# marekrams/tnac4o

Measured on AMD Instinct MI355X. Metric: PEPS-contraction ms/sweep, chimera L=2048 chi=64 (boundary-MPS sweep _setup_rhoT), lower is better.
Workload: dtype f64; 1 GPU; chimera L=2048 (Nx=Ny=16, Nc=8), synthetic couplings seed 20260004, beta=3, chi=64; one sweep = 16 rows of MPO absorb + compress_mps; one step = the sweeps of the 4 lattice rotations of one instance; parallelism=1 GPU: 4 lattice rotations of one instance interleaved on 4 HIP streams, mode=sweep

## Files before the change

include/tnpeps.h:

```cpp
#ifndef TNPEPS_H
#define TNPEPS_H
#include <stdint.h>

#ifdef __cplusplus
extern "C" {
#endif

int tn_version(void);
int tn_build_id(char* buf, int n);
int tn_stream_create_masked(const uint32_t* mask_host, int nwords, void** stream_out);
int tn_stream_destroy(void* stream);
int tn_last_error(char* buf, int n);

int tn_gemm(int64_t M, int64_t N, int64_t K, double alpha, const double* A, int64_t rsa, int64_t csa,
            const double* B, int64_t rsb, int64_t csb, double beta, double* C, int64_t rsc, int64_t csc,
            int64_t batch, int64_t bsa, int64_t bsb, int64_t bsc, void* ws, int64_t ws_bytes, void* stream);
int64_t tn_gemm_ws_bytes(int64_t M, int64_t N, int64_t K, int64_t batch);

int tn_factor_products_eligible(int64_t Z, int64_t I, int64_t J, int64_t K1, int64_t N, int64_t M, int first_batched);
int64_t tn_factor_products_ws_bytes(int64_t Z, int64_t I, int64_t J, int64_t K1, int64_t N, int first_batched);
int tn_factor_products(int64_t Z, int64_t I, int64_t J, int64_t K1, int64_t N, int64_t Mhi, int64_t Mlo, const double* P, int64_t pz,
                       int64_t pi, int64_t pk, const double* X, int64_t xk, int64_t xj, int64_t xn, const double* W, int64_t wm,
                       int64_t wq, double* Out, int64_t oz, int64_t ohi, int64_t olo, int64_t on, int first_batched, void* ws,
                       int64_t ws_bytes, void* stream);

int tn_absorb(const double* A, const double* W, double* out, int64_t Dl, int64_t pold, int64_t Dr, int64_t ba,
              int64_t po, int64_t bb, int64_t pi, int hconj, int64_t batch, int64_t bsA, int64_t bsW, int64_t bsOut,
              void* stream);

int tn_qr(double* A, int64_t rs, int64_t cs, int64_t m, int64_t n, double* Q, int64_t qrs, int64_t qcs, double* R,
          int64_t rrs, int64_t rcs, int nb, double rank_tol, int64_t* keff_host, void* ws, int64_t ws_bytes, void* stream);
int64_t tn_qr_ws_bytes(int64_t m, int64_t n, int nb);
int64_t tn_panel_orth_ws_bytes(int64_t nrows, int b);
int tn_panel_orth(const double* X, int64_t rs, int64_t cs, int64_t nrows, int b, double* Y, int64_t yrs, int64_t ycs, int method,
                  int* state9_host, double* dev_host, void* ws, int64_t ws_bytes, void* stream);
int tn_panel_stats(uint64_t* out16_host, int reset);
int tn_panel_stats_stream(uint64_t* out16_host, int reset, void* stream);
int tn_smallqr_stats(uint64_t* out4_host, int reset, void* stream);
int tn_fused_timeouts(int* count_host, void* stream);
int tn_qr_batched(double* A, int64_t rs, int64_t cs, int64_t m, int64_t n, double* Q, int64_t qrs, int64_t qcs, double* R,
                  int64_t rrs, int64_t rcs, int nb, double rank_tol, int64_t* keff_host, int64_t batch, int64_t bsA, int64_t bsQ,
                  int64_t bsR, void* ws, int64_t ws_bytes, void* stream, void* const* side_streams, int nside);

int tn_svd_trunc(const double* C, int64_t crs, int64_t ccs, int64_t k, int64_t n, int64_t Dmax, double tol, double* U,
                 int64_t urs, int64_t ucs, double* S, double* Vt, int64_t vrs, int64_t vcs, int64_t* keep_host,
                 double* discarded_host, int* sweeps_host, int* info_host, void* ws, int64_t ws_bytes, void* stream);
int tn_svdvals(const double* C, int64_t crs, int64_t ccs, int64_t k, int64_t n, double* S_host, int* sweeps_host,
               int* info_host, void* ws, int64_t ws_bytes, void* stream);
int64_t tn_svd_ws_bytes(int64_t k, int64_t n, int vectors);
int tn_svdvals_async(const double* C, int64_t crs, int64_t ccs, int64_t k, int64_t n, double* out66_dev, void* stream);
int tn_svdvals_small_batched(const int64_t* desc_dev, int64_t batch, const int64_t* desc_host, double* out66_dev, void* stream);
int tn_svd_trunc_batched(const double* C, int64_t crs, int64_t ccs, int64_t k, int64_t n, int64_t Dmax, double tol, double* U,
                         int64_t urs, int64_t ucs, double* S, double* Vt, int64_t vrs, int64_t vcs, int64_t* keep_host,
                         double* discarded_host, int* sweeps_host, int* info_host, int64_t batch, int64_t bsC, int64_t bsU,
                         int64_t bsS, int64_t bsV, void* ws, int64_t ws_bytes, void* stream);
int tn_svdvals_batched(const double* C, int64_t crs, int64_t ccs, int64_t k, int64_t n, double* S_host, int* sweeps_host,
                       int* info_host, int64_t batch, int64_t bsC, void* ws, int64_t ws_bytes, void* stream);

int tn_nfactor(const double* x, int64_t n, double* out2, void* slot8, void* stream);
int tn_normalize_pow2(double* x, int64_t n, double* out2, void* scratch, int64_t scratch_bytes, void* stream);
int tn_scale_by(double* x, int64_t n, const double* scalar_dev, void* stream);
int tn_scale_phys(double* A, int64_t Dl, int64_t p, int64_t Dr, const double* diag, int inv, void* stream);

int tn_peps_factor(const double* Es, const double* E1, const double* E4, const double* Xu, const double* Xl, const double* Xr,
                   const double* Xd, const int32_t* dmap, const int32_t* rmap, int64_t q, int64_t nl, int64_t nu, double* F,
                   void* stream);
int tn_mpo_from_factor(const double* F, const int32_t* dmap, const int32_t* rmap, int64_t q, int64_t nl, int64_t nu, int64_t pd,
                       int64_t br, double* W, void* stream);
int tn_mpo_from_factor_ops(const double* F, const int32_t* dmap, const int32_t* rmap, const double* O, int64_t nop, int64_t q, int64_t nl,
                           int64_t nu, int64_t pd, int64_t br, double* Wops, void* stream);

int tn_calc_pn(const double* T1, const double* RR, const double* F, const int32_t* dmap, const int32_t* rmap,
               const int32_t* pref, const int32_t* suf, const int32_t* lidx, const int32_t* uidx, int64_t nb,
               int64_t q, int64_t nl, int64_t nu, int64_t p, int64_t Dr, int64_t br, double* P, double* minP,
               const double* parent_log2p, double* log2p_out, void* stream);
int tn_sample_pn(const double* T1, const double* RR, const double* F, const int32_t* dmap, const int32_t* rmap, const int32_t* pref,
                 const int32_t* suf, const int32_t* lidx, const int32_t* uidx, const int32_t* perm, const int64_t* starts, int64_t ng,
// ... 161 lines not shown
```

tnac4o_amd/_lib.py:

```python
import ctypes as C
import os
import subprocess

HERE = os.path.dirname(os.path.abspath(__file__))
LIB_PATH = os.path.join(HERE, 'libtnpeps.so')
CSRC = os.path.join(HERE, 'csrc')
SOURCES = ['api.hip', 'gemm_f64.hip', 'rank_update.hip', 'factor_products.hip', 'small.hip', 'qr.hip', 'svd.hip', 'absorb.hip', 'misc.hip', 'beam.hip', 'prof.hip', 'cholqr.hip', 'smallqr.hip', 'fused.hip', 'peps.hip', 'env.hip', 'batch.hip', 'site.hip', 'chain.hip', 'beamsearch.hip', 'marginal.hip', 'sampler.hip', 'overlap.hip', 'relax.hip', 'exchange.hip', 'temper.hip', 'anneal.hip', 'rng.hip', 'droplets.hip', 'linkage.hip', 'lines.hip']

_i64, _f64, _int, _ptr = C.c_int64, C.c_double, C.c_int, C.c_void_p

SIGNATURES = {
    'tn_version': (_int, []),
    'tn_last_error': (_int, [C.c_char_p, _int]),
    'tn_build_id': (_int, [C.c_char_p, _int]),
    'tn_stream_create_masked': (_int, [C.POINTER(C.c_uint32), _int, C.POINTER(_ptr)]),
    'tn_stream_destroy': (_int, [_ptr]),
    'tn_gemm': (_int, [_i64, _i64, _i64, _f64, _ptr, _i64, _i64, _ptr, _i64, _i64, _f64, _ptr, _i64, _i64,
                       _i64, _i64, _i64, _i64, _ptr, _i64, _ptr]),
    'tn_gemm_ws_bytes': (_i64, [_i64, _i64, _i64, _i64]),
    'tn_factor_products_eligible': (_int, [_i64] * 6 + [_int]),
    'tn_factor_products_ws_bytes': (_i64, [_i64] * 5 + [_int]),
    'tn_factor_products': (_int, [_i64] * 7 + [_ptr, _i64, _i64, _i64, _ptr, _i64, _i64, _i64, _ptr, _i64, _i64, _ptr, _i64, _i64, _i64, _i64,
                                  _int, _ptr, _i64, _ptr]),
    'tn_absorb': (_int, [_ptr, _ptr, _ptr, _i64, _i64, _i64, _i64, _i64, _i64, _i64, _int, _i64, _i64, _i64, _i64, _ptr]),
    'tn_qr': (_int, [_ptr, _i64, _i64, _i64, _i64, _ptr, _i64, _i64, _ptr, _i64, _i64, _int, _f64, C.POINTER(_i64), _ptr, _i64,
              _ptr]),
    'tn_qr_ws_bytes': (_i64, [_i64, _i64, _int]),
    'tn_panel_orth_ws_bytes': (_i64, [_i64, _int]),
    'tn_panel_orth': (_int, [_ptr, _i64, _i64, _i64, _int, _ptr, _i64, _i64, _int, C.POINTER(_int), C.POINTER(_f64), _ptr, _i64, _ptr]),
    'tn_panel_stats': (_int, [C.POINTER(C.c_uint64), _int]),
    'tn_panel_stats_stream': (_int, [C.POINTER(C.c_uint64), _int, _ptr]),
    'tn_smallqr_stats': (_int, [C.POINTER(C.c_uint64), _int, _ptr]),
    'tn_fused_timeouts': (_int, [C.POINTER(_int), _ptr]),
    'tn_qr_batched': (_int, [_ptr, _i64, _i64, _i64, _i64, _ptr, _i64, _i64, _ptr, _i64, _i64, _int, _f64, C.POINTER(_i64), _i64, _i64, _i64,
                      _i64, _ptr, _i64, _ptr, C.POINTER(_ptr), _int]),
    'tn_svd_trunc': (_int, [_ptr, _i64, _i64, _i64, _i64, _i64, _f64, _ptr, _i64, _i64, _ptr, _ptr, _i64, _i64,
                            C.POINTER(_i64), C.POINTER(_f64), C.POINTER(_int), C.POINTER(_int), _ptr, _i64, _ptr]),
    'tn_svdvals': (_int, [_ptr, _i64, _i64, _i64, _i64, C.POINTER(_f64), C.POINTER(_int), C.POINTER(_int), _ptr, _i64,
                          _ptr]),
    'tn_svd_ws_bytes': (_i64, [_i64, _i64, _int]),
    'tn_svdvals_async': (_int, [_ptr, _i64, _i64, _i64, _i64, _ptr, _ptr]),
    'tn_svdvals_small_batched': (_int, [_ptr, _i64, _ptr, _ptr, _ptr]),
    'tn_svd_trunc_batched': (_int, [_ptr, _i64, _i64, _i64, _i64, _i64, _f64, _ptr, _i64, _i64, _ptr, _ptr, _i64, _i64, C.POINTER(_i64),
                             C.POINTER(_f64), C.POINTER(_int), C.POINTER(_int), _i64, _i64, _i64, _i64, _i64, _ptr, _i64, _ptr]),
    'tn_svdvals_batched': (_int, [_ptr, _i64, _i64, _i64, _i64, C.POINTER(_f64), C.POINTER(_int), C.POINTER(_int), _i64, _i64, _ptr, _i64,
                           _ptr]),
    'tn_nfactor': (_int, [_ptr, _i64, _ptr, _ptr, _ptr]),
    'tn_scale_by': (_int, [_ptr, _i64, _ptr, _ptr]),
    'tn_normalize_pow2': (_int, [_ptr, _i64, _ptr, _ptr, _i64, _ptr]),
    'tn_scale_phys': (_int, [_ptr, _i64, _i64, _i64, _ptr, _int, _ptr]),
    'tn_calc_pn': (_int, [_ptr] * 9 + [_i64] * 7 + [_ptr, _ptr, _ptr, _ptr, _ptr]),
    'tn_sample_pn': (_int, [_ptr] * 11 + [_i64, _ptr] + [_i64] * 6 + [_ptr, _ptr, _ptr, _ptr]),
    'tn_score_pn': (_int, [_ptr] * 11 + [_i64, _ptr] + [_i64] * 8 + [_ptr, _ptr, _ptr, _ptr, _ptr]),
    'tn_merge_groups': (_int, [_ptr] * 5 + [_i64, _f64, _ptr, _ptr, _ptr, _ptr]),
    'tn_mpo_from_factor_ops': (_int, [_ptr] * 4 + [_i64] * 6 + [_ptr, _ptr]),
    'tn_nfactor_batched': (_int, [_ptr, _i64, _i64, _ptr]),
    'tn_env_rr_batched': (_int, [_ptr] * 5 + [_i64] * 7 + [_ptr, _ptr]),
    'tn_env_rl_batched': (_int, [_ptr] * 3 + [_i64] * 3 + [_ptr, _ptr]),
    'tn_balance': (_int, [_ptr, _i64, _i64, _i64, _f64, _ptr, _ptr, _ptr]),
    'tn_peps_factor': (_int, [_ptr] * 9 + [_i64] * 3 + [_ptr, _ptr]),
    'tn_mpo_from_factor': (_int, [_ptr] * 3 + [_i64] * 5 + [_ptr, _ptr]),
    'tn_site_qr_ws_bytes': (_i64, [_int, _i64, _i64, _i64, _i64, _int]),
    'tn_site_qr': (_int, [_int, _ptr, _i64, _i64, _i64, _ptr, _i64, _ptr, _ptr, _f64, C.POINTER(_i64), _ptr, C.POINTER(_int), C.POINTER(_f64),
                   _int, C.POINTER(_i64), _ptr, _i64, _ptr]),
    'tn_gram_weights': (_int, [_ptr, _i64, _f64, _ptr, _ptr, _ptr]),
    'tn_rows_norm2': (_int, [_ptr, _i64, _i64, _ptr, _ptr]),
    'tn_gather_scale_rows': (_int, [_ptr, _i64, _i64, _ptr, _ptr, _ptr, _int, _ptr]),
    'tn_bond_deflate': (_int, [_int, _ptr, _i64, _i64, _ptr, _i64, _ptr, _ptr, C.POINTER(_i64), C.POINTER(_f64), _ptr, _i64, _ptr]),
    'tn_rar_ws_bytes': (_i64, [_i64] * 5),
    'tn_rar': (_int, [_ptr, _ptr, _ptr] + [_i64] * 5 + [_ptr, _ptr, _i64, _ptr]),
    'tn_env_mix_ws_bytes': (_i64, [_int] + [_i64] * 5),
    'tn_env_mix': (_int, [_int, _ptr, _ptr, _ptr] + [_i64] * 5 + [_ptr, _ptr, _i64, _ptr]),
    'tn_apply_truncation_ws_bytes': (_i64, [_i64] * 5),
    'tn_apply_truncation': (_int, [_ptr, _i64, _i64, _ptr, _i64, _i64, _i64, _ptr, _i64, _i64, _ptr, _i64, _i64, _ptr, _ptr, _ptr, _ptr, _ptr,
                            _i64, _ptr]),
    'tn_compress_mps_arena_bytes': (_i64, [_i64, C.POINTER(_i64), C.POINTER(_i64), _i64]),
# ... 82 lines not shown
    src_hash = source_hash()

    def one(s):
        src = os.path.join(CSRC, s)
        h = hh.copy()
        h.update(open(src, 'rb').read())
        extra = []
        if s == 'api.hip':
            extra = ['-DTN_SRC_HASH="%s"' % src_hash]
            h.update(src_hash.encode())
        obj = os.path.join(objdir, '%s.%s.o' % (s[:-4], h.hexdigest()[:16]))
        if not os.path.exists(obj):
            for old in os.listdir(objdir):
                if old.startswith(s[:-4] + '.') and old.endswith('.o'):
                    os.unlink(os.path.join(objdir, old))
            import tempfile
            fd, tmp = tempfile.mkstemp(prefix=s[:-4] + '.', suffix='.o.part', dir=objdir)
            os.close(fd)
            cmd = [hipcc] + flags + extra + ['-c', src, '-o', tmp]
            if verbose:
                print(' '.join(cmd), flush=True)
            try:
                subprocess.run(cmd, check=True)
                os.replace(tmp, obj)
            finally:
                if os.path.exists(tmp):
                    os.unlink(tmp)
        return obj

    with ThreadPoolExecutor(max_workers=int(os.environ.get('TN_BUILD_JOBS', '6'))) as ex:
        objs = list(ex.map(one, SOURCES))
    cmd = [hipcc, '--offload-arch=gfx950', '-shared', '-fPIC', '-Wl,--no-undefined'] + os.environ.get('TN_EXTRA_HIPCC_FLAGS', '').split() + ['-o', LIB_PATH] + objs
    if verbose:
        print(' '.join(cmd), flush=True)
    subprocess.run(cmd, check=True)
    return LIB_PATH


def _stale(L):
    buf = C.create_string_buffer(64)
    L.tn_build_id.restype, L.tn_build_id.argtypes = _int, [C.c_char_p, _int]
    L.tn_build_id(buf, 64)
    return buf.value.decode() != source_hash()


SHORT_CALLS = ('tn_gemm', 'tn_gemm_ws_bytes', 'tn_qr_ws_bytes', 'tn_svd_ws_bytes', 'tn_absorb', 'tn_nfactor', 'tn_scale_by',
               'tn_normalize_pow2', 'tn_scale_phys', 'tn_calc_pn', 'tn_sample_pn', 'tn_score_pn', 'tn_nfactor_batched', 'tn_env_rr_batched', 'tn_env_rl_batched',
               'tn_balance', 'tn_merge_groups', 'tn_svdvals_async', 'tn_rar', 'tn_rar_ws_bytes', 'tn_env_mix', 'tn_env_mix_ws_bytes',
               'tn_apply_truncation', 'tn_apply_truncation_ws_bytes', 'tn_site_qr_ws_bytes', 'tn_gram_weights', 'tn_argsort_desc', 'tn_weighted_sum', 'tn_rows_norm2', 'tn_gather_scale_rows', 'tn_peps_factor', 'tn_mpo_from_factor', 'tn_env3', 'tn_env3_ws_bytes',
               'tn_cluster_marginal', 'tn_cluster_marginal_ws_bytes', 'tn_cluster_bond_marginal', 'tn_cluster_bond_marginal_ws_bytes',
               'tn_mpo_from_factor_ops', 'tn_env3_stack', 'tn_env3_stack_ws_bytes', 'tn_stack_cell_law', 'tn_stack_cell_law_ws_bytes',
               'tn_last_error')
_lib = None
ABI_VERSION = 25


def lib():
    global _lib
    if _lib is None:
        if not os.path.exists(LIB_PATH):
            raise RuntimeError('libtnpeps.so not found at %s: run `python -c "import __graft_entry__ as g; g.build()"` '
                               '(the HIP library is the only backend; there is no CPU fallback)' % LIB_PATH)
        L = C.CDLL(LIB_PATH)
        L.tn_version.restype = _int
        if not hasattr(L, 'tn_build_id') or (_stale(L) and not os.environ.get('TN_ALLOW_STALE_LIB')):
            raise RuntimeError('libtnpeps.so was built from other sources than csrc/*.hip + include/tnpeps.h in this tree: '
                               'rebuild it with `python -c "import __graft_entry__ as g; g.build()"` -- a stale library can '
                               'disagree with the ctypes signatures declared here')
        if L.tn_version() != ABI_VERSION:
            raise RuntimeError('libtnpeps.so implements C-ABI version %d, this package binds version %d: rebuild the library'
                               % (L.tn_version(), ABI_VERSION))
        if os.environ.get('TN_PYDLL', '1') != '0':
            P = C.PyDLL(LIB_PATH)
            for name in SHORT_CALLS:
                setattr(L, name, getattr(P, name))
            L._pydll = P
        for name, (res, args) in SIGNATURES.items():
            fn = getattr(L, name)
            fn.restype, fn.argtypes = res, args
        _lib = L
    return _lib


class TnError(RuntimeError):
    pass


def check(rc):
    if rc != 0:
        buf = C.create_string_buffer(512)
        lib().tn_last_error(buf, 512)
        raise TnError('libtnpeps error %d: %s' % (rc, buf.value.decode(errors='replace')))
```

tnac4o_amd/csrc/api.hip:

```cpp
#include <stdarg.h>

#include "../../include/tnpeps.h"
#include "common.h"

namespace tn {

static thread_local char g_err[512] = "";

void set_error(const char* fmt, ...) {
    va_list ap;
    va_start(ap, fmt);
    vsnprintf(g_err, sizeof(g_err), fmt, ap);
    va_end(ap);
}
const char* get_error() { return g_err; }

}

using namespace tn;
#define ST ((hipStream_t)stream)

extern "C" {

int tn_version(void) { return 25; }

#ifndef TN_SRC_HASH
#define TN_SRC_HASH "unknown"
#endif
int tn_build_id(char* buf, int n) {
    const char* e = TN_SRC_HASH;
    const int len = (int)strlen(e);
    if (buf && n > 0) {
        const int c = len < n - 1 ? len : n - 1;
        memcpy(buf, e, c);
        buf[c] = 0;
    }
    return len;
}

void tn_profile_enable(unsigned mask) { prof_set_mask(mask); }
void tn_profile_reset(void) { prof_reset(); }
void tn_profile_sample(unsigned every) { prof_set_sample(every); }
int tn_profile_get(int family, uint64_t* calls_host, double* ms_host, double* flops_host, double* bytes_host) {
    TN_CHECK_ARG(family >= 0 && family < PROF_NFAM, "unknown kernel family");
    TN_CHECK_ARG(calls_host && ms_host && flops_host && bytes_host, "null output");
    prof_get(-1, family, calls_host, ms_host, flops_host, bytes_host);
    return 0;
}
int tn_profile_get_phase(int phase, int family, uint64_t* calls_host, double* ms_host, double* flops_host, double* bytes_host) {
    TN_CHECK_ARG(phase >= -1 && phase < PH_N, "unknown phase");
    TN_CHECK_ARG(family >= 0 && family < PROF_NFAM, "unknown kernel family");
    TN_CHECK_ARG(calls_host && ms_host && flops_host && bytes_host, "null output");
    prof_get(phase, family, calls_host, ms_host, flops_host, bytes_host);
    return 0;
}

int tn_stream_create_masked(const uint32_t* mask_host, int nwords, void** stream_out) {
    TN_CHECK_ARG(mask_host && nwords >= 1 && stream_out, "bad arguments");
    hipStream_t st = nullptr;
    const hipError_t e = hipExtStreamCreateWithCUMask(&st, (uint32_t)nwords, mask_host);
    if (e != hipSuccess) return hip_fail(e, "hipExtStreamCreateWithCUMask");
    fused_forms_disable(st);
    *stream_out = (void*)st;
    return 0;
}
int tn_stream_destroy(void* stream) {
    fused_stream_released((hipStream_t)stream);
    const hipError_t e = hipStreamDestroy((hipStream_t)stream);
    return e == hipSuccess ? 0 : hip_fail(e, "hipStreamDestroy");
}

int tn_last_error(char* buf, int n) {
    const char* e = get_error();
    int len = (int)strlen(e);
    if (buf && n > 0) {
        int c = len < n - 1 ? len : n - 1;
        memcpy(buf, e, c);
// ... 312 lines not shown
```

tnac4o_amd/csrc/chain.hip:

```cpp
#include <math.h>
#include <stdlib.h>

#include <cmath>

#include <algorithm>
#include <chrono>
#include <map>
#include <memory>
#include <mutex>
#include <vector>

#include "common.h"

namespace tn {

__global__ __launch_bounds__(256) void permute4_kernel(const double* __restrict__ in, int64_t s0, int64_t s1, int64_t s2, int64_t s3, int64_t n0,
                                                       int64_t n1, int64_t n2, int64_t n3, double* __restrict__ out) {
    const int64_t tot = n0 * n1 * n2 * n3;
    for (int64_t e = (int64_t)blockIdx.x * 256 + threadIdx.x; e < tot; e += (int64_t)gridDim.x * 256) {
        const int64_t i3 = e % n3, r = e / n3, i2 = r % n2, r2 = r / n2, i1 = r2 % n1, i0 = r2 / n1;
        out[e] = in[i0 * s0 + i1 * s1 + i2 * s2 + i3 * s3];
    }
}
static int permute4(hipStream_t st, const double* in, int64_t s0, int64_t s1, int64_t s2, int64_t s3, int64_t n0, int64_t n1, int64_t n2, int64_t n3,
// ... 591 lines not shown
            const double rank_tol = (compress && 0 < n && n < L) ? CH_RANK_TOL : 0.0;
            const M2 Cm = C;
            PassMark tm(st);
            if (compress) tm.substart();
            CH(site_right(n, &Cm, rank_tol));
            if (compress) { tm.trlap(pass_id, 0); trmark = &tm; CH(truncateC(Dmax, tol)); trmark = nullptr; }
        }
        return 0;
    }

    static bool factor_pair_fused(int64_t Z, int64_t I, int64_t J, int64_t K1, int64_t N, int64_t M, int64_t M1, int64_t N1) {
        return factor_products_on() && factor_products_fits(Z, I, J, K1, N, M) && (M1 == 0 || gemm_ws_bytes(M1, N1, K1, 1) == 0);
    }
    int gram_step_structured(M2& G, int64_t n) {
        const int64_t* fd = &facdims[7 * n];
        const int64_t Dl = fd[0], ps = fd[1], Dr = fd[2], ba = fd[3], po = fd[4], bb = fd[5], pi = fd[6];
        const double* Af = facA[n];
        const double* W = facW[n];
        const int64_t wl = po * bb * pi, wr = pi;
        const int64_t wsd = hconj ? bb * pi : 1, wtd = hconj ? 1 : bb * pi;
        const int64_t pt = hconj ? pi : po;
        const int64_t na = Dl * ba;
        Ref gpb; double* Gp = nullptr;
        CH(new_block(na * ba * Dl, gpb, Gp, "Gram (permuted)"));
        if (hconj) CH(permute4(st, G.p, ba * na, na, 1, ba, Dl, ba, ba, Dl, Gp));
        else CH(permute4(st, G.p, na, Dl * na, Dl, 1, Dl, ba, ba, Dl, Gp));
        Ref wxb; double* Wx = nullptr;
        Ref t2b; double* T2 = nullptr;
        if (factor_pair_fused(na, ba, ps, Dl, Dr, pt * bb, na * ba, ps * Dr)) {
            CH(new_block(pt * bb * ba * ps, wxb, Wx, "Wx"));
            CH(permute4(st, W, wl, wsd, wtd, wr, ba, ps, pt, bb, Wx));
            CH(new_block(na * pt * bb * Dr, t2b, T2, "Gram step T2"));
            FactorProducts f;
            f.Z = na; f.I = ba; f.J = ps; f.K1 = Dl; f.N = Dr; f.Mhi = 1; f.Mlo = pt * bb;
            f.P = Gp; f.pz = ba * Dl; f.pi = Dl; f.pk = 1;
            f.X = Af; f.xk = ps * Dr; f.xj = Dr; f.xn = 1;
            f.W = Wx; f.wm = 1; f.wq = pt * bb;
            f.Out = T2; f.oz = pt * bb * Dr; f.ohi = 0; f.olo = Dr; f.on = 1;
            CH(factor_products(st, f));
            gpb.reset();
        } else {
            Ref t1b; double* T1 = nullptr;
            CH(new_block(na * ba * ps * Dr, t1b, T1, "Gram step T1"));
            CH(mm(na * ba, ps * Dr, Dl, Gp, Dl, 1, Af, ps * Dr, 1, T1, ps * Dr, 1));
            gpb.reset();
            CH(new_block(pt * bb * ba * ps, wxb, Wx, "Wx"));
            CH(permute4(st, W, wtd, wr, wl, wsd, pt, bb, ba, ps, Wx));
            CH(new_block(na * pt * bb * Dr, t2b, T2, "Gram step T2"));
            CH(bmm(na, pt * bb, Dr, ba * ps, Wx, ba * ps, 1, 0, T1, Dr, 1, ba * ps * Dr, T2, Dr, 1, pt * bb * Dr));
        }
        Ref wyb; double* Wy = nullptr;
        CH(new_block(ps * bb * ba * pt, wyb, Wy, "Wy"));
        CH(permute4(st, W, wsd, wr, wl, wtd, ps, bb, ba, pt, Wy));
        Ref ub; double* U = nullptr;
        CH(new_block(Dl * ps * bb * bb * Dr, ub, U, "Gram step U"));
        CH(bmm(Dl, ps * bb, bb * Dr, ba * pt, Wy, ba * pt, 1, 0, T2, bb * Dr, 1, ba * pt * bb * Dr, U, bb * Dr, 1, ps * bb * bb * Dr));
        t2b.reset();
        Ref ob; double* O = nullptr;
        CH(new_block(Dr * bb * bb * Dr, ob, O, "Gram step O"));
        CH(mm(Dr, bb * bb * Dr, Dl * ps, Af, 1, Dr, U, bb * bb * Dr, 1, O, bb * bb * Dr, 1));
        ub.reset();
        M2 Gn;
        CH(new_m2(Dr * bb, Dr * bb, Gn, "Gram matrix"));
        if (hconj) CH(permute4(st, O, bb * bb * Dr, bb * Dr, 1, Dr, Dr, bb, Dr, bb, Gn.p));
        else CH(permute4(st, O, bb * Dr, bb * bb * Dr, Dr, 1, bb, Dr, bb, Dr, Gn.p));
        G = Gn;
        return 0;
    }
    int ensure_absorbed(int64_t n) {
        if (A[n].p) return 0;
        if (facA.empty() || !facA[n]) { set_error("tn_compress_mps: site %lld has neither a tensor nor its factors", (long long)n); return -1; }
        const int64_t* fd = &facdims[7 * n];
        T3 t;
        CH(new_t3(A[n].a, A[n].b, A[n].c, t, "absorbed site"));
        {
            ProfPhase ph(PH_ABSORB);
            CH(absorb(st, facA[n], facW[n], t.p, fd[0], fd[1], fd[2], fd[3], fd[4], fd[5], fd[6], hconj, 1, 0, 0, 0));
        }
        A[n] = t;
        return 0;
    }
    int attach_through_factors(int64_t n, const M2& Cm, double* Am) {
        const int64_t* fd = &facdims[7 * n];
        const int64_t Dl = fd[0], ps = fd[1], Dr = fd[2], ba = fd[3], po = fd[4], bb = fd[5], pi = fd[6], r = Cm.c;
        const int64_t pt = hconj ? pi : po;
        if (Cm.r != Dr * bb || (hconj ? po : pi) != ps) { set_error("tn_compress_mps: centre matrix does not fit the factors of site %lld", (long long)n); return -1; }
        if (factor_pair_fused(Dl, ps, bb, Dr, r, ba * pt, hconj ? Dl * ps : 0, bb * r)) {
            Ref wb; double* Wq = nullptr;
            CH(new_block(ba * pt * ps * bb, wb, Wq, "attach through the factors: W"));
            if (hconj) CH(permute4(st, facW[n], bb * pi, pi, po * bb * pi, 1, ps, bb, ba, pt, Wq));
            else CH(permute4(st, facW[n], 1, pi, po * bb * pi, bb * pi, ps, bb, ba, pt, Wq));
            FactorProducts f;
            f.Z = Dl; f.I = ps; f.J = bb; f.K1 = Dr; f.N = r; f.Mhi = ba; f.Mlo = pt;
            f.P = facA[n]; f.pz = ps * Dr; f.pi = Dr; f.pk = 1;
            f.X = Cm.p; f.xk = hconj ? bb * r : r; f.xj = hconj ? r : Dr * r; f.xn = 1;
            f.W = Wq; f.wm = 1; f.wq = ba * pt;
            f.Out = Am; f.oz = hconj ? ba * pt * r : pt * r; f.ohi = hconj ? pt * r : Dl * pt * r; f.olo = r; f.on = 1;
            return factor_products(st, f);
        }
        Ref tb; double* T = nullptr;
        CH(new_block(Dl * ps * bb * r, tb, T, "attach through the factors: T"));
        if (hconj) CH(mm(Dl * ps, bb * r, Dr, facA[n], Dr, 1, Cm.p, bb * r, 1, T, bb * r, 1));
        else CH(bmm(bb, Dl * ps, r, Dr, facA[n], Dr, 1, 0, Cm.p, r, 1, Dr * r, T, bb * r, 1, r));
        Ref wb; double* Wq = nullptr;
        CH(new_block(ba * pt * ps * bb, wb, Wq, "attach through the factors: W"));
        if (hconj) CH(permute4(st, facW[n], po * bb * pi, 1, bb * pi, pi, ba, pt, ps, bb, Wq));
// ... 504 lines not shown
    pm.lap(5);
    if ((rc = ch.variational_compress(*target, tolV, max_sweeps, lazy))) return rc;
    pm.lap(6);
    for (int64_t n = 0; n < L; ++n) {
        const T3& t = ch.A[n];
        TN_CHECK_ARG(t.numel() <= out_slot, "output slot too small for a compressed site");
        const hipError_t e = hipMemcpyAsync(out + n * out_slot, t.p, (size_t)t.numel() * 8, hipMemcpyDeviceToDevice, st);
        if (e != hipSuccess) return hip_fail(e, "copy result");
        out_dims_host[3 * n] = t.a; out_dims_host[3 * n + 1] = t.b; out_dims_host[3 * n + 2] = t.c;
    }
    pm.lap(7);
    if (overlap_host) *overlap_host = ch.overlap;
    if (discarded_host) for (int64_t i = 0; i <= L; ++i) discarded_host[i] = ch.discarded[i];
    if (schmidt_host && schmidt_len_host) {
        for (int64_t i = 0; i <= L; ++i) {
            Chain::SState& s = ch.Sst[i];
            if (s.is_lazy) {
                std::vector<double> v;
                if ((rc = ch.svdvals_host(s.lazy, v))) return rc;
                s.val = v; s.has = true; s.is_lazy = false; s.lazy = M2();
            }
            const int64_t len = s.has ? std::min<int64_t>((int64_t)s.val.size(), schmidt_pitch) : 0;
            schmidt_len_host[i] = s.has ? len : -1;
            for (int64_t j = 0; j < len; ++j) schmidt_host[i * schmidt_pitch + j] = s.val[j];
        }
    }
    if (ch.nfs_overflow) {
        set_error("tn_compress_mps: the table of normalisation factors is too small (%lld pairs): size it (2 max_sweeps + 16) L + 64", (long long)nfs_cap);
        return -3;
    }
    if (nfs_count_host) *nfs_count_host = ch.nfs_count;
    if (info_host) {
        info_host[0] = ch.reveal_error_bound;
        info_host[1] = (double)ch.reveal_fallbacks;
        info_host[2] = (double)ch.weighted_used;
        info_host[3] = (double)ar.peak();
        info_host[4] = (double)ch.bonds_before;
        info_host[5] = (double)ch.bonds_after;
        info_host[6] = 0.0;
        info_host[7] = (double)ch.gauge_skipped + 65536.0 * (double)ch.target_swapped + 131072.0 * (double)ch.var1_skipped + 262144.0 * (double)ch.attach_fused;
    }
    return 0;
}

int tn_argsort_desc(const double* w, int64_t n, int64_t* perm_out, void* stream) {
    TN_CHECK_ARG(w && perm_out, "null operand");
    return argsort_desc((hipStream_t)stream, w, n, perm_out);
}
int tn_weighted_sum(const double* a, const double* b, int64_t n, double* w_out, double* sum_out, void* stream) {
    TN_CHECK_ARG(a && b && w_out && sum_out, "null operand");
    return weighted_sum((hipStream_t)stream, a, b, n, w_out, sum_out);
}

}
```

tnac4o_amd/csrc/common.h:

```cpp
#pragma once
#include <hip/hip_runtime.h>
#include <stdint.h>
#include <stdio.h>
#include <stdlib.h>
#include <string.h>

namespace tn {

void set_error(const char* fmt, ...);
const char* get_error();

inline int hip_fail(hipError_t e, const char* what) {
    set_error("%s: %s", what, hipGetErrorString(e));
    return (int)e > 0 ? (int)e : 1;
}

#define TN_CHECK_ARG(cond, msg)                \
    do {                                       \
        if (!(cond)) {                         \
            tn::set_error("%s: %s", __func__, msg); \
            return -1;                         \
        }                                      \
    } while (0)

// ... 74 lines not shown
void prof_set_sample(unsigned n);
void prof_reset();
void prof_get(int phase, int fam, uint64_t* calls, double* ms, double* flops, double* bytes);

struct Mat {
    double* p;
    int64_t rs, cs;
};
static inline Mat mat(double* p, int64_t rs, int64_t cs) { return Mat{p, rs, cs}; }
static inline Mat sub(Mat a, int64_t i, int64_t j) { return Mat{a.p + i * a.rs + j * a.cs, a.rs, a.cs}; }
static inline Mat tr(Mat a) { return Mat{a.p, a.cs, a.rs}; }

int gemm(hipStream_t st, int64_t M, int64_t N, int64_t K, double alpha, const double* A, int64_t rsa, int64_t csa,
         const double* B, int64_t rsb, int64_t csb, double beta, double* C, int64_t rsc, int64_t csc,
         int64_t batch = 1, int64_t bsa = 0, int64_t bsb = 0, int64_t bsc = 0, double* ws = nullptr,
         int64_t ws_bytes = 0);
int64_t gemm_ws_bytes(int64_t M, int64_t N, int64_t K, int64_t batch);
struct GemmExtra {
    const int* pairs = nullptr;
    const int* skip = nullptr;
    int pw = 0, mapA = 0, mapB = 0, mapC = 0;
    int force_splitk = 0;
    bool raw_partials = false;
    int* splitk_used = nullptr;
};
int gemm_forced_split(int64_t K, int s, int64_t* kchunk);
int gemm_ex(hipStream_t st, int64_t M, int64_t N, int64_t K, double alpha, const double* A, int64_t rsa, int64_t csa,
            const double* B, int64_t rsb, int64_t csb, double beta, double* C, int64_t rsc, int64_t csc, int64_t batch,
            int64_t bsa, int64_t bsb, int64_t bsc, double* ws, int64_t ws_bytes, const GemmExtra* x);

static inline int gemm(hipStream_t st, int64_t M, int64_t N, int64_t K, double alpha, Mat A, Mat B, double beta, Mat C,
                       double* ws = nullptr, int64_t ws_bytes = 0) {
    return gemm(st, M, N, K, alpha, A.p, A.rs, A.cs, B.p, B.rs, B.cs, beta, C.p, C.rs, C.cs, 1, 0, 0, 0, ws, ws_bytes);
}
int gemm_prof_family(int64_t M, int64_t N, int64_t K, int64_t rsc, int64_t csc);

int rank_update(hipStream_t st, int64_t m, int64_t n, int b, const double* W, int64_t wrs, int64_t wcs, const double* X, int64_t xrs,
                int64_t xcs, double* C, int64_t rsc, int64_t csc, const int* active);
static inline int rank_update(hipStream_t st, int64_t m, int64_t n, int b, Mat W, Mat X, Mat C, const int* active = nullptr) {
    return rank_update(st, m, n, b, W.p, W.rs, W.cs, X.p, X.rs, X.cs, C.p, C.rs, C.cs, active);
}

struct FactorProducts {
    int64_t Z, I, J, K1, N, Mhi, Mlo;
    const double* P; int64_t pz, pi, pk;
    const double* X; int64_t xk, xj, xn;
    const double* W; int64_t wm, wq;
    double* Out; int64_t oz, ohi, olo, on;
};
bool factor_products_fits(int64_t Z, int64_t I, int64_t J, int64_t K1, int64_t N, int64_t M);
inline bool factor_products_on() { return env_flag_on("TN_FACTOR_FUSED"); }
int factor_products(hipStream_t st, const FactorProducts& f);

constexpr int NBMAX = 64;

int gram_partial(hipStream_t st, const double* X, int64_t vs, int64_t es, int64_t L, int nvec, int w, const int* pairs,
                 int ngroups, int nchunk, double* part);
int gram_nchunk(int64_t L);

int eig_small(hipStream_t st, const double* part, int nchunk, int nvec, int ngroups, int mode, int max_sweeps,
              double dead_thresh, double* out, int* dead, int* nrot, double* maxoff, double relevant2 = 0.0, int allow_fast = 1);

int rows_times_small(hipStream_t st, double* X, int64_t rs, int64_t cs, int64_t nrows, int b, const double* S);

struct SvdRoundsJob {
    double* X; int64_t pitch, L; int nvp, w;
    const int* pairs; int ng, nr, nchunk;
    double* part; int64_t part_bytes; double* Js; int* nrot; double* maxoff;
    double relevant2, last_tol; int inner_first, inner_later;
    double* norms;
};
int svd_rounds_fused(hipStream_t st, const SvdRoundsJob& j);
int small_t_times_vecs(hipStream_t st, const double* S, double* X, int64_t vs, int64_t es, int64_t L, int nvec, int w,
                       const int* pairs, int ngroups, const int* nrot);


int qr_factor(hipStream_t st, double* A, int64_t rs, int64_t cs, int64_t m, int64_t n, double* Q, int64_t qrs, int64_t qcs, double* R,
              int64_t rrs, int64_t rcs, int nb, void* ws, int64_t ws_bytes, double rank_tol, int64_t* keff_host,
              double* dropped2_host = nullptr, int frob_exit = 0, int64_t* pivot_perm_host = nullptr, double* nf_out2 = nullptr,
              int* nf_done = nullptr);
int64_t qr_ws_bytes(int64_t m, int64_t n, int nb);


constexpr int CQ_MAXPASS = 4;
constexpr double CQ_THETA = 1e-10;
constexpr double CQ_DONE = 5e-15;
constexpr double CQ_LAST = 1e-8;
int64_t cholqr_ws_bytes(int64_t nrows, int b);
int cholqr_reset(hipStream_t st, void* ws);
int cholqr_begin(hipStream_t st, void* ws, void** state_out);
void cholqr_end_ok(hipStream_t st);
int cholqr_orthonormalize(hipStream_t st, const double* X, int64_t irs, int64_t ics, double* Y, int64_t rs, int64_t cs, int64_t nrows,
                          int b, void* ws, int64_t ws_bytes, uint64_t seed, int* fused_base, void* state = nullptr);
int cholqr_panel(hipStream_t st, const double* X, int64_t irs, int64_t ics, double* Y, int64_t rs, int64_t cs, int64_t nrows, int b, void* ws,
                 int64_t ws_bytes, uint64_t seed, int reconstruct, double* Tp, double* W, int64_t wrs, int64_t wcs, double* Wq, int* fused_base,
                 void* state = nullptr, const int* active = nullptr);
int cholqr_debug_state(hipStream_t st, const void* ws, int* ints9, double* dev_hist);
int cholqr_stats(unsigned long long* out16, int reset, hipStream_t st_or_null, int all_streams);
bool smallqr_fits(int64_t m, int64_t n);
int64_t smallqr_ws_bytes(int64_t m, int64_t n);
int smallqr_factor(hipStream_t st, const double* A, int64_t rs, int64_t cs, int64_t m, int64_t n, double* Q, int64_t qrs, int64_t qcs, double* R,
                   int64_t rrs, int64_t rcs, double* nf_out2, void* ws, int64_t ws_bytes);

constexpr int CQ_FUSED_MAXBLK = 32;
constexpr unsigned CQ_SPIN_LIMIT = 1u << 22;
constexpr int CHOLQR_SLOTS = 64;
// ... 110 lines not shown
```

Measured before the change: 368.9 ms/sweep.

## Fuse Gram-step batched GEMM, contraction and permute into one MFMA kernel

Adds a gram_products kernel that computes the Gram matrix in the chain Gram step directly. The Wy×T2 product and the contraction with A are chained per alpha in registers and LDS, and the result is written straight into the permuted output layout. This removes the large intermediate U buffer, the second GEMM launch and the permute pass. It uses f64 MFMA with double-buffered LDS staging of T2 and A. The cost is that each row-group block reloads T2 for every alpha, and the path only applies when shapes fit the kernel limits and the GEMM needs no workspace.

```diff
diff --git a/include/tnpeps.h b/include/tnpeps.h
--- a/include/tnpeps.h
+++ b/include/tnpeps.h
@@ -23,6 +23,11 @@
                        int64_t pi, int64_t pk, const double* X, int64_t xk, int64_t xj, int64_t xn, const double* W, int64_t wm,
                        int64_t wq, double* Out, int64_t oz, int64_t ohi, int64_t olo, int64_t on, int first_batched, void* ws,
                        int64_t ws_bytes, void* stream);
+
+int tn_gram_products_eligible(int64_t Dl, int64_t ps, int64_t Dr, int64_t bb, int64_t Q);
+int64_t tn_gram_products_ws_bytes(int64_t Dl, int64_t ps, int64_t Dr, int64_t bb, int64_t Q);
+int tn_gram_products(int64_t Dl, int64_t ps, int64_t Dr, int64_t bb, int64_t Q, const double* Wy, const double* T2, const double* A,
+                     double* Gn, int hconj, void* ws, int64_t ws_bytes, void* stream);
 
 int tn_absorb(const double* A, const double* W, double* out, int64_t Dl, int64_t pold, int64_t Dr, int64_t ba,
               int64_t po, int64_t bb, int64_t pi, int hconj, int64_t batch, int64_t bsA, int64_t bsW, int64_t bsOut,
diff --git a/tnac4o_amd/_lib.py b/tnac4o_amd/_lib.py
--- a/tnac4o_amd/_lib.py
+++ b/tnac4o_amd/_lib.py
@@ -5,7 +5,7 @@
 HERE = os.path.dirname(os.path.abspath(__file__))
 LIB_PATH = os.path.join(HERE, 'libtnpeps.so')
 CSRC = os.path.join(HERE, 'csrc')
-SOURCES = ['api.hip', 'gemm_f64.hip', 'rank_update.hip', 'factor_products.hip', 'small.hip', 'qr.hip', 'svd.hip', 'absorb.hip', 'misc.hip', 'beam.hip', 'prof.hip', 'cholqr.hip', 'smallqr.hip', 'fused.hip', 'peps.hip', 'env.hip', 'batch.hip', 'site.hip', 'chain.hip', 'beamsearch.hip', 'marginal.hip', 'sampler.hip', 'overlap.hip', 'relax.hip', 'exchange.hip', 'temper.hip', 'anneal.hip', 'rng.hip', 'droplets.hip', 'linkage.hip', 'lines.hip']
+SOURCES = ['api.hip', 'gemm_f64.hip', 'rank_update.hip', 'factor_products.hip', 'gram_products.hip', 'small.hip', 'qr.hip', 'svd.hip', 'absorb.hip', 'misc.hip', 'beam.hip', 'prof.hip', 'cholqr.hip', 'smallqr.hip', 'fused.hip', 'peps.hip', 'env.hip', 'batch.hip', 'site.hip', 'chain.hip', 'beamsearch.hip', 'marginal.hip', 'sampler.hip', 'overlap.hip', 'relax.hip', 'exchange.hip', 'temper.hip', 'anneal.hip', 'rng.hip', 'droplets.hip', 'linkage.hip', 'lines.hip']
 
 _i64, _f64, _int, _ptr = C.c_int64, C.c_double, C.c_int, C.c_void_p
 
@@ -22,6 +22,9 @@
     'tn_factor_products_ws_bytes': (_i64, [_i64] * 5 + [_int]),
     'tn_factor_products': (_int, [_i64] * 7 + [_ptr, _i64, _i64, _i64, _ptr, _i64, _i64, _i64, _ptr, _i64, _i64, _ptr, _i64, _i64, _i64, _i64,
                                   _int, _ptr, _i64, _ptr]),
+    'tn_gram_products_eligible': (_int, [_i64] * 5),
+    'tn_gram_products_ws_bytes': (_i64, [_i64] * 5),
+    'tn_gram_products': (_int, [_i64] * 5 + [_ptr, _ptr, _ptr, _ptr, _int, _ptr, _i64, _ptr]),
     'tn_absorb': (_int, [_ptr, _ptr, _ptr, _i64, _i64, _i64, _i64, _i64, _i64, _i64, _int, _i64, _i64, _i64, _i64, _ptr]),
     'tn_qr': (_int, [_ptr, _i64, _i64, _i64, _i64, _ptr, _i64, _i64, _ptr, _i64, _i64, _int, _f64, C.POINTER(_i64), _ptr, _i64,
               _ptr]),
@@ -210,7 +213,7 @@
                'tn_mpo_from_factor_ops', 'tn_env3_stack', 'tn_env3_stack_ws_bytes', 'tn_stack_cell_law', 'tn_stack_cell_law_ws_bytes',
                'tn_last_error')
 _lib = None
-ABI_VERSION = 25
+ABI_VERSION = 26
 
 
 def lib():
diff --git a/tnac4o_amd/csrc/api.hip b/tnac4o_amd/csrc/api.hip
--- a/tnac4o_amd/csrc/api.hip
+++ b/tnac4o_amd/csrc/api.hip
@@ -22,7 +22,7 @@
 
 extern "C" {
 
-int tn_version(void) { return 25; }
+int tn_version(void) { return 26; }
 
 #ifndef TN_SRC_HASH
 #define TN_SRC_HASH "unknown"
diff --git a/tnac4o_amd/csrc/chain.hip b/tnac4o_amd/csrc/chain.hip
--- a/tnac4o_amd/csrc/chain.hip
+++ b/tnac4o_amd/csrc/chain.hip
@@ -667,6 +667,18 @@
         Ref wyb; double* Wy = nullptr;
         CH(new_block(ps * bb * ba * pt, wyb, Wy, "Wy"));
         CH(permute4(st, W, wsd, wr, wl, wtd, ps, bb, ba, pt, Wy));
+        if (gram_products_on() && gram_products_eligible(Dl, ps, Dr, bb, ba * pt)) {
+            M2 Gn;
+            CH(new_m2(Dr * bb, Dr * bb, Gn, "Gram matrix"));
+            GramProducts f;
+            f.Dl = Dl; f.ps = ps; f.Dr = Dr; f.bb = bb; f.Q = ba * pt;
+            f.Wy = Wy; f.T2 = T2; f.A = Af; f.Out = Gn.p;
+            if (hconj) { f.ob = bb * Dr * bb; f.orr = Dr * bb; f.onl = bb; f.onh = 1; }
+            else { f.orr = Dr * bb * Dr; f.ob = bb * Dr; f.onh = Dr; f.onl = 1; }
+            CH(gram_products(st, f));
+            G = Gn;
+            return 0;
+        }
         Ref ub; double* U = nullptr;
         CH(new_block(Dl * ps * bb * bb * Dr, ub, U, "Gram step U"));
         CH(bmm(Dl, ps * bb, bb * Dr, ba * pt, Wy, ba * pt, 1, 0, T2, bb * Dr, 1, ba * pt * bb * Dr, U, bb * Dr, 1, ps * bb * bb * Dr));
@@ -1277,4 +1289,41 @@
     return weighted_sum((hipStream_t)stream, a, b, n, w_out, sum_out);
 }
 
-}
+int tn_gram_products_eligible(int64_t Dl, int64_t ps, int64_t Dr, int64_t bb, int64_t Q) { return gram_products_eligible(Dl, ps, Dr, bb, Q) ? 1 : 0; }
+static int64_t gram_products_layout(char* base, int64_t Dl, int64_t ps, int64_t Dr, int64_t bb, double** U, double** O, double** gw, int64_t* gw_bytes) {
+    WsCarve c{base};
+    *gw_bytes = gemm_ws_bytes(Dr, bb * bb * Dr, Dl * ps, 1);
+    *U = c.take<double>(Dl * ps * bb * bb * Dr * 8);
+    *O = c.take<double>(Dr * bb * bb * Dr * 8);
+    *gw = c.take<double>(*gw_bytes);
+    return c.total();
+}
+int64_t tn_gram_products_ws_bytes(int64_t Dl, int64_t ps, int64_t Dr, int64_t bb, int64_t Q) {
+    (void)Q;
+    double* U; double* O; double* gw; int64_t gb;
+    return gram_products_layout(nullptr, Dl, ps, Dr, bb, &U, &O, &gw, &gb);
+}
+int tn_gram_products(int64_t Dl, int64_t ps, int64_t Dr, int64_t bb, int64_t Q, const double* Wy, const double* T2, const double* A, double* Gn,
+                     int hconj, void* ws, int64_t ws_bytes, void* stream) {
+    TN_CHECK_ARG(Dl >= 1 && ps >= 1 && Dr >= 1 && bb >= 1 && Q >= 1, "non-positive dimension");
+    TN_CHECK_ARG(Wy && T2 && A && Gn, "null operand");
+    const hipStream_t st = (hipStream_t)stream;
+    if (gram_products_on() && gram_products_eligible(Dl, ps, Dr, bb, Q)) {
+        GramProducts f;
+        f.Dl = Dl; f.ps = ps; f.Dr = Dr; f.bb = bb; f.Q = Q;
+        f.Wy = Wy; f.T2 = T2; f.A = A; f.Out = Gn;
+        if (hconj) { f.ob = bb * Dr * bb; f.orr = Dr * bb; f.onl = bb; f.onh = 1; }
+        else { f.orr = Dr * bb * Dr; f.ob = bb * Dr; f.onh = Dr; f.onl = 1; }
+        return gram_products(st, f);
+    }
+    double* U; double* O; double* gw; int64_t gb;
+    const int64_t need = gram_products_layout((char*)ws, Dl, ps, Dr, bb, &U, &O, &gw, &gb);
+    TN_CHECK_ARG(ws && ws_bytes >= need, "workspace too small (tn_gram_products_ws_bytes)");
+    int rc = gemm(st, ps * bb, bb * Dr, Q, 1.0, Wy, Q, 1, T2, bb * Dr, 1, 0.0, U, bb * Dr, 1, Dl, 0, Q * bb * Dr, ps * bb * bb * Dr, nullptr, 0);
+    if (rc == 0) rc = gemm(st, Dr, bb * bb * Dr, Dl * ps, 1.0, A, 1, Dr, U, bb * bb * Dr, 1, 0.0, O, bb * bb * Dr, 1, 1, 0, 0, 0, gw, gb);
+    if (rc) return rc;
+    if (hconj) return permute4(st, O, bb * bb * Dr, bb * Dr, 1, Dr, Dr, bb, Dr, bb, Gn);
+    return permute4(st, O, bb * Dr, bb * bb * Dr, Dr, 1, bb, Dr, bb, Dr, Gn);
+}
+
+}
diff --git a/tnac4o_amd/csrc/common.h b/tnac4o_amd/csrc/common.h
--- a/tnac4o_amd/csrc/common.h
+++ b/tnac4o_amd/csrc/common.h
@@ -150,6 +150,20 @@
 inline bool factor_products_on() { return env_flag_on("TN_FACTOR_FUSED"); }
 int factor_products(hipStream_t st, const FactorProducts& f);
 
+struct GramProducts {
+    int64_t Dl, ps, Dr, bb, Q;
+    const double* Wy;
+    const double* T2;
+    const double* A;
+    double* Out; int64_t ob, orr, onh, onl;
+};
+bool gram_products_fits(int64_t Dl, int64_t ps, int64_t Dr, int64_t bb, int64_t Q);
+inline bool gram_products_on() { return env_flag_on("TN_GRAM_FUSED"); }
+inline bool gram_products_eligible(int64_t Dl, int64_t ps, int64_t Dr, int64_t bb, int64_t Q) {
+    return gram_products_fits(Dl, ps, Dr, bb, Q) && gemm_ws_bytes(Dr, bb * bb * Dr, Dl * ps, 1) == 0;
+}
+int gram_products(hipStream_t st, const GramProducts& f);
+
 constexpr int NBMAX = 64;
 
 int gram_partial(hipStream_t st, const double* X, int64_t vs, int64_t es, int64_t L, int nvec, int w, const int* pairs,
diff --git a/tnac4o_amd/csrc/gram_products.hip b/tnac4o_amd/csrc/gram_products.hip
--- /dev/null
+++ b/tnac4o_amd/csrc/gram_products.hip
@@ -0,0 +1,168 @@
+#include "common.h"
+
+namespace tn {
+
+namespace {
+
+typedef double d4 __attribute__((ext_vector_type(4)));
+
+constexpr int GP_R = 4;
+constexpr int GP_THREADS = 64 * GP_R;
+constexpr int GP_QMAX = 256;
+constexpr int GP_PSMAX = 16;
+constexpr int GP_DRMAX = 64;
+
+struct GramP {
+    const double* Wy;
+    const double* T2;
+    const double* A;
+    double* Out;
+    int Dl, ps, Dr, bb, Q, N, rgroups;
+    int64_t ob, orr, onh, onl;
+};
+
+template <int NQ>
+__global__ __launch_bounds__(GP_THREADS) void gram_products_kernel(GramP g) {
+    constexpr int KG = 16 * NQ;
+    constexpr int TE = 64 * NQ * 16 / GP_THREADS;
+    constexpr int AE = GP_PSMAX * GP_DRMAX / GP_THREADS;
+    constexpr int TSZ = 64 * NQ * 16, STAGE = TSZ + GP_PSMAX * GP_DRMAX;
+    constexpr int BB = 8;
+    __shared__ double Ls[2][STAGE];
+    const int tid = threadIdx.x, lane = tid & 63, wave = __builtin_amdgcn_readfirstlane(tid >> 6);
+    const int lr = lane & 15, lk = lane >> 4;
+    int bid = blockIdx.x;
+    {
+        const int nwg = gridDim.x, q = nwg / 8, r = nwg % 8, xcd = bid % 8, loc = bid / 8;
+        bid = (xcd < r ? xcd * (q + 1) : r * (q + 1) + (xcd - r) * q) + loc;
+    }
+    const int nt = bid / g.rgroups, rg = bid - nt * g.rgroups;
+    const int n0 = nt * 16, r = rg * GP_R + wave;
+
+    double wy[KG];
+    {
+        const bool row = lr < g.ps && r < g.bb;
+        const double* Wr = g.Wy + ((int64_t)min(lr, g.ps - 1) * g.bb + min(r, g.bb - 1)) * g.Q;
+#pragma unroll
+        for (int kk = 0; kk < KG; ++kk) {
+            const int q = kk * 4 + lk;
+            wy[kk] = Wr[min(q, g.Q - 1)];
+        }
+        __builtin_amdgcn_sched_barrier(0);
+#pragma unroll
+        for (int kk = 0; kk < KG; ++kk) wy[kk] = (row && kk * 4 + lk < g.Q) ? wy[kk] : 0.0;
+    }
+    const int sc = tid & 15, sq = tid >> 4, ab = tid & 63, as = tid >> 6;
+    const bool scv = n0 + sc < g.N, abv = ab < g.Dr;
+    const double* Tp = g.T2 + min(n0 + sc, g.N - 1);
+    const double* Ap = g.A + min(ab, g.Dr - 1);
+    auto gload = [&](double (&t)[TE], double (&a)[AE], const int alpha) {
+        const int ac = min(alpha, g.Dl - 1);
+        const double* Ta = Tp + (int64_t)ac * g.Q * g.N;
+#pragma unroll
+        for (int i = 0; i < TE; ++i) {
+            const int q = i * (GP_THREADS / 16) + sq;
+            t[i] = Ta[(int64_t)min(q, g.Q - 1) * g.N];
+        }
+        const double* Aa = Ap + (int64_t)ac * g.ps * g.Dr;
+#pragma unroll
+        for (int i = 0; i < AE; ++i) {
+            const int s = i * (GP_THREADS / 64) + as;
+            a[i] = Aa[min(s, g.ps - 1) * g.Dr];
+        }
+    };
+    auto lwrite = [&](double* buf, const double (&t)[TE], const double (&a)[AE]) {
+#pragma unroll
+        for (int i = 0; i < TE; ++i) buf[i * GP_THREADS + tid] = (scv && i * (GP_THREADS / 16) + sq < g.Q) ? t[i] : 0.0;
+#pragma unroll
+        for (int i = 0; i < AE; ++i) buf[TSZ + i * GP_THREADS + tid] = (abv && i * (GP_THREADS / 64) + as < g.ps) ? a[i] : 0.0;
+    };
+
+    d4 acc[4];
+#pragma unroll
+    for (int bt = 0; bt < 4; ++bt) acc[bt] = d4{0.0, 0.0, 0.0, 0.0};
+    double t[TE], a[AE];
+    gload(t, a, 0);
+    __builtin_amdgcn_sched_barrier(0);
+    lwrite(Ls[0], t, a);
+    __syncthreads();
+    for (int alpha = 0; alpha < g.Dl; ++alpha) {
+        const double* cur = Ls[alpha & 1] + lk * 16 + lr;
+        const double* ca = Ls[alpha & 1] + TSZ + lk * 64 + lr;
+        gload(t, a, alpha + 1);
+        double b[2][BB];
+#pragma unroll
+        for (int j = 0; j < BB; ++j) b[0][j] = cur[j * 64];
+        __builtin_amdgcn_sched_barrier(0);
+        d4 s = d4{0.0, 0.0, 0.0, 0.0};
+        double af[4][4];
+#pragma unroll
+        for (int k0 = 0; k0 < KG; k0 += BB) {
+            const int c = (k0 / BB) & 1;
+            if (k0 + BB < KG) {
+#pragma unroll
+                for (int j = 0; j < BB; ++j) b[c ^ 1][j] = cur[(k0 + BB + j) * 64];
+            } else {
+#pragma unroll
+                for (int gs = 0; gs < 4; ++gs)
+#pragma unroll
+                    for (int bt = 0; bt < 4; ++bt) af[gs][bt] = ca[gs * 256 + bt * 16];
+            }
+            __builtin_amdgcn_sched_barrier(0);
+#pragma unroll
+            for (int j = 0; j < BB; ++j) s = __builtin_amdgcn_mfma_f64_16x16x4f64(wy[k0 + j], b[c][j], s, 0, 0, 0);
+            __builtin_amdgcn_sched_barrier(0);
+        }
+#pragma unroll
+        for (int gs = 0; gs < 4; ++gs)
+#pragma unroll
+            for (int bt = 0; bt < 4; ++bt) acc[bt] = __builtin_amdgcn_mfma_f64_16x16x4f64(af[gs][bt], s[gs], acc[bt], 0, 0, 0);
+        __builtin_amdgcn_sched_barrier(0);
+        lwrite(Ls[(alpha + 1) & 1], t, a);
+        __syncthreads();
+    }
+
+    const int n = n0 + lr;
+    if (r >= g.bb || n >= g.N) return;
+    const int nh = n / g.Dr, nl = n - nh * g.Dr;
+    double* o = g.Out + (int64_t)r * g.orr + (int64_t)nh * g.onh + (int64_t)nl * g.onl;
+#pragma unroll
+    for (int bt = 0; bt < 4; ++bt)
+#pragma unroll
+        for (int i = 0; i < 4; ++i) {
+            const int beta = bt * 16 + lk + 4 * i;
+            if (beta < g.Dr) o[(int64_t)beta * g.ob] = acc[bt][i];
+        }
+}
+
+}
+
+bool gram_products_fits(int64_t Dl, int64_t ps, int64_t Dr, int64_t bb, int64_t Q) {
+    if (Dl < 1 || ps < 1 || Dr < 1 || bb < 1 || Q < 1) return false;
+    if (ps > GP_PSMAX || ps % 4 != 0 || Q > GP_QMAX || Dr > GP_DRMAX) return false;
+    return Dl < ((int64_t)1 << 30) && bb < ((int64_t)1 << 20) && cdiv(bb * Dr, 16) * cdiv(bb, GP_R) < ((int64_t)1 << 31);
+}
+
+int gram_products(hipStream_t st, const GramProducts& f) {
+    TN_CHECK_ARG(gram_products_fits(f.Dl, f.ps, f.Dr, f.bb, f.Q), "shape outside the kernel's limits");
+    GramP g;
+    g.Wy = f.Wy; g.T2 = f.T2; g.A = f.A; g.Out = f.Out;
+    g.Dl = (int)f.Dl; g.ps = (int)f.ps; g.Dr = (int)f.Dr; g.bb = (int)f.bb; g.Q = (int)f.Q; g.N = (int)(f.bb * f.Dr);
+    g.rgroups = (int)cdiv(f.bb, GP_R);
+    g.ob = f.ob; g.orr = f.orr; g.onh = f.onh; g.onl = f.onl;
+    const dim3 grid((unsigned)(cdiv(g.N, 16) * g.rgroups));
+    const double N = (double)g.N, K2 = (double)(f.Dl * f.ps);
+    prof_begin(st, PROF_GEMM_64x64);
+    switch (cdiv(f.Q, 64)) {
+        case 1: hipLaunchKernelGGL((gram_products_kernel<1>), grid, dim3(GP_THREADS), 0, st, g); break;
+        case 2: hipLaunchKernelGGL((gram_products_kernel<2>), grid, dim3(GP_THREADS), 0, st, g); break;
+        case 3: hipLaunchKernelGGL((gram_products_kernel<3>), grid, dim3(GP_THREADS), 0, st, g); break;
+        default: hipLaunchKernelGGL((gram_products_kernel<4>), grid, dim3(GP_THREADS), 0, st, g); break;
+    }
+    TN_CHECK_LAUNCH("gram_products_kernel");
+    prof_end(st, PROF_GEMM_64x64, 2.0 * f.bb * N * K2 * ((double)f.Q + (double)f.Dr),
+             8.0 * ((double)f.ps * f.bb * f.Q + (double)g.rgroups * f.Dl * f.Q * N + K2 * f.Dr + (double)f.Dr * f.bb * N));
+    return 0;
+}
+
+}
```

Result: slower. 390.9 ms/sweep (+6.0%).
